# mmbajo/PROBA-V

Measured on AMD Instinct MI355X. Metric: LR-patches/sec fwd+bwd (WDSR-B r12 t9, 16x16, bs128), higher is better.
Workload: dtype f32 (products as 3 scaled-fp16-piece MFMA products, f32 accumulate)

## Files before the change

### proba-v_amd/csrc/kernels_direct.hip

```cpp
#include "probav_common.h"
#include "x6_device.h"

namespace probav {

__device__ __forceinline__ int reflect_idx(int i, int n) {
    i = i < 0 ? -i : i;
    return i >= n ? 2 * n - 2 - i : i;
}

template <int COUT_T, int VEC>
__global__ __launch_bounds__(256) void conv_direct_fwd_kernel(
    ConvGeom g, const float* __restrict__ x, const float* __restrict__ gate, const float* __restrict__ w,
    const float* __restrict__ bias, const float* __restrict__ skip, float* __restrict__ y)
{
    const long nvox = (long)g.N * g.Ho * g.Wo * g.To;
    const long v = (long)blockIdx.x * 256 + threadIdx.x;
    if (v >= nvox) return;
    const int co0 = blockIdx.y * COUT_T;
    long r = v;
    const int t = (int)(r % g.To); r /= g.To;
    const int wo = (int)(r % g.Wo); r /= g.Wo;
    const int h = (int)(r % g.Ho);
    const int n = (int)(r / g.Ho);

// ... 7 lines not shown
        if (g.reflect_hw) ih = reflect_idx(ih, g.Hi);
        else if (ih < 0 || ih >= g.Hi) { pad_h = true; ih = 0; }
        for (int b = 0; b < g.kw; ++b) {
            int iw = wo + b - g.pw;
            bool pad_w = pad_h;
            if (g.reflect_hw) iw = reflect_idx(iw, g.Wi);
            else if (iw < 0 || iw >= g.Wi) { pad_w = true; iw = 0; }
            for (int c = 0; c < g.kt; ++c) {
                int it = t + c - g.pt;
                bool pad = pad_w;
                if (g.reflect_t) it = reflect_idx(it, g.Ti);
                else if (it < 0 || it >= g.Ti) { pad = true; it = 0; }
                const long vin = (((long)n * g.Hi + ih) * g.Wi + iw) * g.Ti + it;
                const float* xp = x + vin * g.Cin;
                const float* gp = gate ? gate + vin * g.Cin : nullptr;
                const float* wp = w + (long)((a * g.kw + b) * g.kt + c) * g.Cin * g.Cout + co0;
                for (int ci = 0; ci < g.Cin; ci += VEC) {
                    float xv[VEC];
                    if constexpr (VEC == 4) {
                        const float4 q = *reinterpret_cast<const float4*>(xp + ci);
                        xv[0] = q.x; xv[1] = q.y; xv[2] = q.z; xv[3] = q.w;
                        if (gp) {
                            const float4 m = *reinterpret_cast<const float4*>(gp + ci);
                            xv[0] = m.x > 0.f ? xv[0] : 0.f; xv[1] = m.y > 0.f ? xv[1] : 0.f;
                            xv[2] = m.z > 0.f ? xv[2] : 0.f; xv[3] = m.w > 0.f ? xv[3] : 0.f;
                        }
                    } else {
                        xv[0] = xp[ci];
                        if (gp) xv[0] = gp[ci] > 0.f ? xv[0] : 0.f;
                    }
#pragma unroll
                    for (int u = 0; u < VEC; ++u) {
                        if (pad) xv[u] = 0.f;
                        const float* wr = wp + (long)(ci + u) * g.Cout;
#pragma unroll
                        for (int j = 0; j < COUT_T; ++j) acc[j] = fmaf(xv[u], wr[j], acc[j]);
                    }
                }
            }
        }
    }
    float* yp = y + v * g.Cout + co0;
    const float* sp = skip ? skip + v * g.Cout + co0 : nullptr;
#pragma unroll
    for (int j = 0; j < COUT_T; ++j) {
        float o = acc[j] + (bias ? bias[co0 + j] : 0.f);
        if (g.relu) o = relu_keep_nan(o);
        if (sp) o += sp[j];
        yp[j] = o;
    }
}

template <int COUT_T>
static int launch_fwd(const ConvGeom& g, const float* x, const float* gate, const float* w, const float* bias,
                      const float* skip, float* y, hipStream_t s)
{
    const long nvox = (long)g.N * g.Ho * g.Wo * g.To;
    dim3 grid((unsigned)((nvox + 255) / 256), (unsigned)(g.Cout / COUT_T));
    const bool vec4 = (g.Cin % 4 == 0) && ((reinterpret_cast<uintptr_t>(x) & 15) == 0) &&
                      (!gate || (reinterpret_cast<uintptr_t>(gate) & 15) == 0);
    if (vec4) hipLaunchKernelGGL((conv_direct_fwd_kernel<COUT_T, 4>), grid, dim3(256), 0, s, g, x, gate, w, bias, skip, y);
    else      hipLaunchKernelGGL((conv_direct_fwd_kernel<COUT_T, 1>), grid, dim3(256), 0, s, g, x, gate, w, bias, skip, y);
    return check_launch("conv_direct_fwd");
}

constexpr int C1_ROWS = 4;
__global__ __launch_bounds__(256) void conv3_cin1_fwd_kernel(ConvGeom g, const float* __restrict__ x, const float* __restrict__ w,
                                                            const float* __restrict__ bias, float* __restrict__ y, unsigned* __restrict__ amax)
{
    extern __shared__ float c1_in[];
    const int tid = threadIdx.x, cg = tid & 7, vs = tid >> 3;
    const int Wp = g.Wi + 2, Tp = g.Ti + 2, nin = 3 * Wp * Tp, nv = g.Wo * g.To;
    float4 wt[27];
#pragma unroll
    for (int k = 0; k < 27; ++k) wt[k] = *reinterpret_cast<const float4*>(w + k * 32 + 4 * cg);
    const float4 b4 = bias ? *reinterpret_cast<const float4*>(bias + 4 * cg) : make_float4(0.f, 0.f, 0.f, 0.f);
    const unsigned mT = 0xffffffffu / (unsigned)g.To + 1u, mTp = 0xffffffffu / (unsigned)Tp + 1u, mWT = 0xffffffffu / (unsigned)(Wp * Tp) + 1u;
    const long nrows = (long)g.N * g.Ho;
    float omax = 0.f;
    int n_prev = -1;
#pragma unroll 1
    for (int r = 0; r < C1_ROWS; ++r) {
        const long R = (long)blockIdx.x * C1_ROWS + r;
        if (R >= nrows) break;
        const int n = (int)(R / g.Ho), h = (int)(R - (long)n * g.Ho);
        if (n != n_prev) { if (amax && n_prev >= 0) amax_commit(omax, amax + n_prev); omax = 0.f; n_prev = n; }
        __syncthreads();
        for (int i = tid; i < nin; i += 256) {
            const int dh = (int)__umulhi((unsigned)i, mWT), rem = i - dh * Wp * Tp;
            const int wp = (int)__umulhi((unsigned)rem, mTp), tp = rem - wp * Tp;
            const int ih = h - 1 + dh, iw = wp - 1, it = tp - 1;
            const bool ok = ih >= 0 && ih < g.Hi && iw >= 0 && iw < g.Wi && it >= 0 && it < g.Ti;
            c1_in[i] = ok ? x[(((long)n * g.Hi + ih) * g.Wi + iw) * g.Ti + it] : 0.f;
        }
        __syncthreads();
        float* yrow = y + ((long)n * g.Ho + h) * nv * 32;
        for (int v = vs; v < nv; v += 32) {
            const int wo = (int)__umulhi((unsigned)v, mT), t = v - wo * g.To;
            const float* ip = c1_in + wo * Tp + t;
            float4 acc = b4;
#pragma unroll
            for (int dh = 0; dh < 3; ++dh)
#pragma unroll
                for (int dw = 0; dw < 3; ++dw)
#pragma unroll
                    for (int dt = 0; dt < 3; ++dt) {
                        const float xv = ip[(dh * Wp + dw) * Tp + dt];
                        const float4 q = wt[(dh * 3 + dw) * 3 + dt];
                        acc.x = fmaf(xv, q.x, acc.x); acc.y = fmaf(xv, q.y, acc.y); acc.z = fmaf(xv, q.z, acc.z); acc.w = fmaf(xv, q.w, acc.w);
                    }
            if (g.relu) { acc.x = relu_keep_nan(acc.x); acc.y = relu_keep_nan(acc.y); acc.z = relu_keep_nan(acc.z); acc.w = relu_keep_nan(acc.w); }
            *reinterpret_cast<float4*>(yrow + (long)v * 32 + 4 * cg) = acc;
            omax = fmaxf(fmaxf(omax, fmaxf(fabsf(acc.x), fabsf(acc.y))), fmaxf(fabsf(acc.z), fabsf(acc.w)));
        }
    }
    if (amax && n_prev >= 0) amax_commit(omax, amax + n_prev);
}

bool conv3d_cin1_forward_supported(const ConvGeom& g)
{
    return g.Cin == 1 && g.Cout == 32 && g.kh == 3 && g.kw == 3 && g.kt == 3 && g.ph == 1 && g.pw == 1 && g.pt == 1 && !g.reflect_hw && !g.reflect_t &&
           g.Ho == g.Hi && g.Wo == g.Wi && g.To == g.Ti && g.To >= 2 && (g.Wi + 2) * (g.Ti + 2) * 3 * sizeof(float) <= 48 * 1024;
}
int conv3d_cin1_forward(const ConvGeom& g, const float* x, const float* w, const float* bias, float* y, unsigned* amax, hipStream_t s)
{
    if (!conv3d_cin1_forward_supported(g)) { set_error("conv3d_cin1_forward: unsupported geometry", hipSuccess); return PROBAV_EINVAL; }
    const long nrows = (long)g.N * g.Ho;
    const size_t lds = (size_t)3 * (g.Wi + 2) * (g.Ti + 2) * sizeof(float);
    hipLaunchKernelGGL(conv3_cin1_fwd_kernel, dim3((unsigned)((nrows + C1_ROWS - 1) / C1_ROWS)), dim3(256), lds, s, g, x, w, bias, y, amax);
    return check_launch("conv3_cin1_fwd");
}

int conv3d_direct_forward(const ConvGeom& g, const float* x, const float* gate, const float* w,
                          const float* bias, const float* skip, float* y, hipStream_t s)
{
    if (g.N <= 0) return PROBAV_OK;
    if (g.Cout % 32 == 0) return launch_fwd<32>(g, x, gate, w, bias, skip, y, s);
    if (g.Cout % 25 == 0) return launch_fwd<25>(g, x, gate, w, bias, skip, y, s);
    if (g.Cout % 9 == 0)  return launch_fwd<9>(g, x, gate, w, bias, skip, y, s);
    if (g.Cout % 4 == 0)  return launch_fwd<4>(g, x, gate, w, bias, skip, y, s);
    return launch_fwd<1>(g, x, gate, w, bias, skip, y, s);
}

bool conv3d_up_forward_supported(const ConvGeom& g)
{
    return g.Cin == 32 && g.Cout == 9 && g.kh == 3 && g.kw == 3 && g.kt == 3 && g.ph == 0 && g.pw == 0 && g.pt == 0 && !g.reflect_hw && !g.reflect_t &&
           g.Ti == 3 && g.To == 1 && g.Ho == g.Hi - 2 && g.Wo == g.Wi - 2 && g.Wo == 16;
}
bool conv3d_up_bwd_data_supported(const ConvGeom& g)
{
    return g.Cin == 9 && g.Cout == 32 && g.kh == 3 && g.kw == 3 && g.kt == 3 && g.ph == 2 && g.pw == 2 && g.pt == 2 && !g.reflect_hw && !g.reflect_t &&
           g.Ti == 1 && g.To == 3 && g.Ho == g.Hi + 2 && g.Wo == g.Wi + 2 && g.Wi <= 30;
}
__global__ __launch_bounds__(256) void conv3_up_fwd_kernel(ConvGeom g, const float* __restrict__ x, const float* __restrict__ w,
                                                          const float* __restrict__ bias, float* __restrict__ y)
{
    extern __shared__ float up_lds[];
    float* sW = up_lds;
    float* sX = sW + 27 * 32 * 9;
    const int tid = threadIdx.x;
    const int rowf = g.Wi * 3 * 32;
    if ((reinterpret_cast<unsigned long>(w) & 15) == 0) {
        for (int i = tid; i < 27 * 32 * 9 / 4; i += 256) reinterpret_cast<float4*>(sW)[i] = reinterpret_cast<const float4*>(w)[i];
    } else {
        for (int i = tid; i < 27 * 32 * 9; i += 256) sW[i] = w[i];
    }
    const int wo = tid >> 4, kp = tid & 15;
    for (int row = blockIdx.x; row < g.N * g.Ho; row += gridDim.x) {
    const int n = row / g.Ho, h = row - n * g.Ho;
    __syncthreads();
    const float4* xr = reinterpret_cast<const float4*>(x + ((long)n * g.Hi + h) * rowf);
    for (int i = tid; i < 3 * rowf / 4; i += 256) reinterpret_cast<float4*>(sX)[i] = xr[i];
    __syncthreads();
    float acc[9];
#pragma unroll
    for (int j = 0; j < 9; ++j) acc[j] = 0.f;
#pragma unroll 2
    for (int q = 0; q < 54; ++q) {
        const int k = kp + 16 * q;
        const int tap = k >> 5, ci = k & 31;
        const int a = tap / 9, bc = tap - 9 * a, b = bc / 3, c = bc - 3 * b;
        const float xv = sX[a * rowf + ((wo + b) * 3 + c) * 32 + ci];
        const float* wr = sW + k * 9;
#pragma unroll
        for (int j = 0; j < 9; ++j) acc[j] = fmaf(xv, wr[j], acc[j]);
    }
#pragma unroll
    for (int j = 0; j < 9; ++j) {
        float v = acc[j];
#pragma unroll
        for (int m = 1; m < 16; m <<= 1) v += __shfl_xor(v, m, 64);
        acc[j] = v;
    }
    if (kp < 9) {
        float o = 0.f;
#pragma unroll
        for (int j = 0; j < 9; ++j) o = kp == j ? acc[j] : o;
        o += bias ? bias[kp] : 0.f;
        if (g.relu) o = relu_keep_nan(o);
        y[(((long)n * g.Ho + h) * g.Wo + wo) * 9 + kp] = o;
    }
    }
}
__global__ __launch_bounds__(256) void conv3_up_bwd_data_kernel(ConvGeom g, const float* __restrict__ dy, const float* __restrict__ wT,
                                                               const float* __restrict__ bias, float* __restrict__ dx, unsigned* __restrict__ amax)
{
    extern __shared__ float up_lds[];
    float* sW = up_lds;
    float* sD = sW + 27 * 9 * 32;
    const int tid = threadIdx.x;
    const int Wp = g.Wi + 4;
    if ((reinterpret_cast<unsigned long>(wT) & 15) == 0) {
        for (int i = tid; i < 27 * 9 * 32 / 4; i += 256) reinterpret_cast<float4*>(sW)[i] = reinterpret_cast<const float4*>(wT)[i];
    } else {
        for (int i = tid; i < 27 * 9 * 32; i += 256) sW[i] = wT[i];
    }
    __shared__ float red[4];
    for (int row = blockIdx.x; row < g.N * g.Ho; row += gridDim.x) {
    const int n = row / g.Ho, h = row - n * g.Ho;
    __syncthreads();
    for (int i = tid; i < 3 * Wp * 9; i += 256) {
        const int a = i / (Wp * 9), r = i - a * Wp * 9, wp = r / 9, co = r - 9 * wp;
        const int ih = h + a - 2, iw = wp - 2;
        sD[i] = (ih >= 0 && ih < g.Hi && iw >= 0 && iw < g.Wi) ? dy[(((long)n * g.Hi + ih) * g.Wi + iw) * 9 + co] : 0.f;
    }
    __syncthreads();
    float omax = 0.f;
    const int items = g.Wo * 3 * 8;
    for (int it = tid; it < items; it += 256) {
        const int cg = it & 7, wt = it >> 3, wo = wt / 3, t = wt - 3 * wo;
        float4 acc = bias ? make_float4(bias[4 * cg], bias[4 * cg + 1], bias[4 * cg + 2], bias[4 * cg + 3]) : make_float4(0.f, 0.f, 0.f, 0.f);
#pragma unroll
        for (int a = 0; a < 3; ++a)
#pragma unroll
            for (int b = 0; b < 3; ++b) {
                const float* dp = sD + (a * Wp + wo + b) * 9;
                const float* wp = sW + (((a * 3 + b) * 3 + (2 - t)) * 9) * 32 + 4 * cg;
#pragma unroll
                for (int co = 0; co < 9; ++co) {
                    const float d = dp[co];
                    const float4 q = *reinterpret_cast<const float4*>(wp + co * 32);
                    acc.x = fmaf(d, q.x, acc.x); acc.y = fmaf(d, q.y, acc.y); acc.z = fmaf(d, q.z, acc.z); acc.w = fmaf(d, q.w, acc.w);
                }
            }
        *reinterpret_cast<float4*>(dx + ((((long)n * g.Ho + h) * g.Wo + wo) * 3 + t) * 32 + 4 * cg) = acc;
        omax = fmaxf(fmaxf(omax, fmaxf(fabsf(acc.x), fabsf(acc.y))), fmaxf(fabsf(acc.z), fabsf(acc.w)));
    }
    if (amax) {
#pragma unroll
        for (int o = 32; o; o >>= 1) omax = fmaxf(omax, __shfl_xor(omax, o, 64));
        if ((tid & 63) == 0) red[tid >> 6] = omax;
        __syncthreads();
        if (tid == 0) {
            const float m = fmaxf(fmaxf(red[0], red[1]), fmaxf(red[2], red[3]));
            atomicMax(amax + n, __float_as_uint(m));
        }
    }
    }
}
int conv3d_up_forward(const ConvGeom& g, const float* x, const float* w, const float* bias, float* y, hipStream_t s)
{
    if (!conv3d_up_forward_supported(g)) { set_error("conv3d_up_forward: unsupported geometry", hipSuccess); return PROBAV_EINVAL; }
    const size_t lds = ((size_t)27 * 32 * 9 + (size_t)3 * g.Wi * 3 * 32) * sizeof(float);
    hipLaunchKernelGGL(conv3_up_fwd_kernel, dim3((unsigned)(g.N * g.Ho < 512 ? g.N * g.Ho : 512)), dim3(256), lds, s, g, x, w, bias, y);
    return check_launch("conv3_up_fwd");
}
int conv3d_up_bwd_data(const ConvGeom& g, const float* dy, const float* wT, const float* bias, float* dx, unsigned* amax, hipStream_t s)
{
    if (!conv3d_up_bwd_data_supported(g)) { set_error("conv3d_up_bwd_data: unsupported geometry", hipSuccess); return PROBAV_EINVAL; }
    const size_t lds = ((size_t)27 * 9 * 32 + (size_t)3 * (g.Wi + 4) * 9) * sizeof(float);
    hipLaunchKernelGGL(conv3_up_bwd_data_kernel, dim3((unsigned)(g.N * g.Ho < 768 ? g.N * g.Ho : 768)), dim3(256), lds, s, g, dy, wT, bias, dx, amax);
    return check_launch("conv3_up_bwd_data");
}

template <int KH, int KW, int KT, int CI_PER>
__global__ __launch_bounds__(256) void conv_direct_wgrad_kernel(
    ConvGeom g, const float* __restrict__ x, const float* __restrict__ dy, const float* __restrict__ gate,
    float* __restrict__ partial, float* __restrict__ partial_b, long vox_per_chunk)
{
    constexpr int TAPS = KH * KW * KT;
    const int tid = threadIdx.x;
    const int co = blockIdx.y * 32 + (tid & 31);
    const bool co_ok = co < g.Cout;
    const int ci0 = (blockIdx.z * 8 + (tid >> 5)) * CI_PER;
    const long nvox = (long)g.N * g.Ho * g.Wo * g.To;
    const long v0 = (long)blockIdx.x * vox_per_chunk;
    const long v1 = v0 + vox_per_chunk < nvox ? v0 + vox_per_chunk : nvox;

    float acc[TAPS][CI_PER];
#pragma unroll
    for (int tp = 0; tp < TAPS; ++tp)
#pragma unroll
        for (int k = 0; k < CI_PER; ++k) acc[tp][k] = 0.f;
    float accb = 0.f;
    const bool vec4 = (CI_PER % 4 == 0) && (g.Cin % 4 == 0) && (ci0 + CI_PER <= g.Cin);

    for (long v = v0; v < v1; ++v) {
        long r = v;
        const int t = (int)(r % g.To); r /= g.To;
        const int wo = (int)(r % g.Wo); r /= g.Wo;
        const int h = (int)(r % g.Ho);
        const int n = (int)(r / g.Ho);
        float d = 0.f;
        if (co_ok) {
            d = dy[v * g.Cout + co];
            if (gate) d = gate[v * g.Cout + co] > 0.f ? d : 0.f;
        }
        accb += d;
#pragma unroll
        for (int a = 0; a < KH; ++a) {
            int ih = h + a - g.ph;
            if (g.reflect_hw) ih = reflect_idx(ih, g.Hi);
            else if (ih < 0 || ih >= g.Hi) continue;
#pragma unroll
            for (int b = 0; b < KW; ++b) {
                int iw = wo + b - g.pw;
                if (g.reflect_hw) iw = reflect_idx(iw, g.Wi);
                else if (iw < 0 || iw >= g.Wi) continue;
#pragma unroll
                for (int c = 0; c < KT; ++c) {
                    int it = t + c - g.pt;
                    if (g.reflect_t) it = reflect_idx(it, g.Ti);
                    else if (it < 0 || it >= g.Ti) continue;
                    const float* xp = x + ((((long)n * g.Hi + ih) * g.Wi + iw) * g.Ti + it) * g.Cin + ci0;
                    const int tp = (a * KW + b) * KT + c;
                    bool done = false;
                    if constexpr (CI_PER % 4 == 0) {
                        if (vec4) {
#pragma unroll
                            for (int k = 0; k < CI_PER; k += 4) {
                                const float4 q = *reinterpret_cast<const float4*>(xp + k);
                                acc[tp][k] = fmaf(q.x, d, acc[tp][k]);
                                acc[tp][k + 1] = fmaf(q.y, d, acc[tp][k + 1]);
                                acc[tp][k + 2] = fmaf(q.z, d, acc[tp][k + 2]);
                                acc[tp][k + 3] = fmaf(q.w, d, acc[tp][k + 3]);
                            }
                            done = true;
                        }
                    }
                    if (!done) {
#pragma unroll
                        for (int k = 0; k < CI_PER; ++k)
                            if (ci0 + k < g.Cin) acc[tp][k] = fmaf(xp[k], d, acc[tp][k]);
                    }
                }
            }
        }
    }
    if (co_ok) {
        float* pp = partial + (long)blockIdx.x * TAPS * g.Cin * g.Cout;
#pragma unroll
        for (int tp = 0; tp < TAPS; ++tp)
#pragma unroll
            for (int k = 0; k < CI_PER; ++k)
                if (ci0 + k < g.Cin) pp[((long)tp * g.Cin + ci0 + k) * g.Cout + co] = acc[tp][k];
        if (blockIdx.z == 0 && (tid >> 5) == 0) partial_b[(long)blockIdx.x * g.Cout + co] = accb;
    }
}

static int sum_partials(const float* p1, float* o1, long n1, const float* p2, float* o2, long n2, int chunks, hipStream_t s)
{
    SlabSumJob jobs[2] = {{p1, o1, n1, (int)n1, chunks}, {p2, o2, n2, (int)n2, chunks}};
    return slab_sum_later(s, jobs, o2 ? 2 : 1);
}


__global__ __launch_bounds__(1024) void wgrad2d_small_kernel(ConvGeom g, const float* __restrict__ x, const float* __restrict__ dy,
                                                            const float* __restrict__ gate, float* __restrict__ partial,
                                                            float* __restrict__ partial_b, int halves)
{
    extern __shared__ float lds2d[];
    const int tid = threadIdx.x, nthr = blockDim.x;
    const int n = blockIdx.x / halves, part = blockIdx.x - n * halves;
    const int r0 = part * g.Ho / halves, r1 = (part + 1) * g.Ho / halves;
    const int nrow_o = r1 - r0, nrow_i = nrow_o + 2;
    float* xs = lds2d;
    float* ds = xs + nrow_i * g.Wi * g.Cin;
    const float* xsrc = x + ((long)n * g.Hi + r0) * g.Wi * g.Cin;
    for (int i = tid; i < nrow_i * g.Wi * g.Cin; i += nthr) xs[i] = xsrc[i];
    const long dbase = ((long)n * g.Ho + r0) * g.Wo * g.Cout;
    for (int i = tid; i < nrow_o * g.Wo * g.Cout; i += nthr) {
        float d = dy[dbase + i];
        if (gate) d = gate[dbase + i] > 0.f ? d : 0.f;
        ds[i] = d;
    }
    __syncthreads();
    const int nout = 9 * g.Cin * g.Cout;
    const long slab = (long)nout + g.Cout;
    float* pp = partial + (long)blockIdx.x * nout;
    if (tid < nout) {
        const int co = tid % g.Cout, rest = tid / g.Cout, ci = rest % g.Cin, tap = rest / g.Cin;
        const int a = tap / 3, b = tap - 3 * a;
        const float* xp = xs + (a * g.Wi + b) * g.Cin + ci;
        const float* dp = ds + co;
        float acc = 0.f;
        for (int h = 0; h < nrow_o; ++h)
            for (int w = 0; w < g.Wo; ++w) acc = fmaf(xp[(h * g.Wi + w) * g.Cin], dp[(h * g.Wo + w) * g.Cout], acc);
        pp[tid] = acc;
    } else if (tid < nout + g.Cout) {
        const int co = tid - nout;
        float acc = 0.f;
        for (int i = 0; i < nrow_o * g.Wo; ++i) acc += ds[i * g.Cout + co];
        partial_b[(long)blockIdx.x * g.Cout + co] = acc;
    }
    (void)slab;
}

static bool small2d(const ConvGeom& g, int& halves, size_t& lds)
{
    if (g.kh != 3 || g.kw != 3 || g.kt != 1 || g.Ti != 1 || g.To != 1 || g.ph || g.pw || g.pt || g.reflect_hw) return false;
    if (9 * g.Cin * g.Cout + g.Cout > 1024 || g.Ho < 2) return false;
    halves = 2;
    const int nrow_o = (g.Ho + 1) / 2 + 1;
    lds = ((size_t)(nrow_o + 2) * g.Wi * g.Cin + (size_t)nrow_o * g.Wo * g.Cout) * sizeof(float);
    return lds <= 64 * 1024;
}

static void wgrad_plan(const ConvGeom& g, int& ci_per, int& gy, int& gz, int& chunks, long& vpc)
{
    const bool k3d = (g.kh == 3 && g.kw == 3 && g.kt == 3);
    const bool k2d = (g.kh == 3 && g.kw == 3 && g.kt == 1);
    if (g.kh == 5) ci_per = 1;
    else if (k3d) ci_per = g.Cin >= 4 ? 4 : 1;
// ... 312 lines not shown
```

### proba-v_amd/csrc/kernels_loss.hip

```cpp
#include "probav_common.h"
#include "reduce_device.h"

namespace probav {

__device__ __forceinline__ double corrected(double p, double bias, double m) { return (p + bias) * m; }
__device__ __forceinline__ double residual(double h, double p, double bias, double m) { return h - corrected(p, bias, m); }

struct Crop {
    const float* H; const uint8_t* M; const float* P;
    int S, border, L, i, j;
    __device__ __forceinline__ bool clear(int r, int c) const { return M[(i + r) * S + j + c] != 0; }
    __device__ __forceinline__ float hr(int r, int c) const { return H[(i + r) * S + j + c]; }
    __device__ __forceinline__ float pred(int r, int c) const { return P[(border + r) * S + border + c]; }
    __device__ __forceinline__ double m(int r, int c) const { return clear(r, c) ? 1.0 : 0.0; }
    __device__ __forceinline__ double residual(int r, int c, double bias) const { return probav::residual((double)hr(r, c), (double)pred(r, c), bias, m(r, c)); }
};
__device__ __forceinline__ Crop crop_at(const float* hr, const uint8_t* mask, const float* pred, int b, int S, int border, int i, int j)
{
    const long o = (long)b * S * S;
    return Crop{hr + o, mask + o, pred + o, S, border, S - 2 * border, i, j};
}
__device__ __forceinline__ Crop crop_of_shift(const float* hr, const uint8_t* mask, const float* pred, int b, int S, int border, int sft)
{
    const int ns = 2 * border + 1, i = sft / ns;
    return crop_at(hr, mask, pred, b, S, border, i, sft - i * ns);
}

__device__ __forceinline__ void crop_walk(const Crop& x, int tid, double& cnt, double& dsum)
{
    cnt = 0.0; dsum = 0.0;
    for (int k = tid; k < x.L * x.L; k += 256) {
        const int r = k / x.L, c = k - r * x.L;
        const float m = x.clear(r, c) ? 1.f : 0.f;
        cnt += (double)m;
        dsum += (double)(x.hr(r, c) - x.pred(r, c) * m);
    }
}
__device__ __forceinline__ double crop_bias(const Crop& x, int tid, double* red, double& cnt)
{
    double dsum;
    crop_walk(x, tid, cnt, dsum);
    cnt = block_sum(cnt, red, tid);
    dsum = block_sum(dsum, red, tid);
    return dsum / cnt;
}

struct FirstMin {
    double best = 1e300;
    int arg = 0;
    __device__ __forceinline__ void take(double v, int sft) { if (v < best) { best = v; arg = sft; } }
    __device__ __forceinline__ double value() const { return best < 1e300 ? best : __builtin_nan(""); }
};

__global__ __launch_bounds__(256) void shift_loss_fwd_kernel(
    const float* __restrict__ hr, const uint8_t* __restrict__ mask, const float* __restrict__ pred, int S, int border,
    double* __restrict__ cand)
{
    const int b = blockIdx.x, i = blockIdx.y, lane = threadIdx.x & 63, wave = threadIdx.x >> 6;
    const int L = S - 2 * border, ns = 2 * border + 1, nshift = ns * ns;
    for (int j = wave; j < ns; j += 4) {
        const int sft = i * ns + j;
        const Crop x = crop_at(hr, mask, pred, b, S, border, i, j);
        constexpr int U = 4;
        const int n = L * L;
        double cnt = 0.0, dsum = 0.0;
        for (int k0 = lane; k0 < n; k0 += 64 * U) {
            float m[U], h[U], q[U];
#pragma unroll
            for (int u = 0; u < U; ++u) {
                const int k = k0 + 64 * u < n ? k0 + 64 * u : k0;
                const int r = k / L, c = k - r * L;
                m[u] = x.clear(r, c) ? 1.f : 0.f;
                h[u] = x.hr(r, c);
                q[u] = x.pred(r, c);
            }
#pragma unroll
            for (int u = 0; u < U; ++u)
                if (k0 + 64 * u < n) { cnt += (double)m[u]; dsum += (double)(h[u] - q[u] * m[u]); }
        }
        cnt = wave_sum(cnt); dsum = wave_sum(dsum);
        const double bias = dsum / cnt;
        double s1 = 0.0, s2 = 0.0;
        for (int k0 = lane; k0 < n; k0 += 64 * U) {
            float h[U], q[U]; bool mk[U];
#pragma unroll
            for (int u = 0; u < U; ++u) {
                const int k = k0 + 64 * u < n ? k0 + 64 * u : k0;
                const int r = k / L, c = k - r * L;
                mk[u] = x.clear(r, c);
                h[u] = x.hr(r, c);
                q[u] = x.pred(r, c);
            }
#pragma unroll
            for (int u = 0; u < U; ++u)
                if (k0 + 64 * u < n) {
                    const double e = residual((double)h[u], (double)q[u], bias, mk[u] ? 1.0 : 0.0);
                    s1 += fabs(e);
                    s2 += e * e;
                }
        }
        s1 = wave_sum(s1) / cnt; s2 = wave_sum(s2) / cnt;
        if (lane == 0) { cand[((long)b * nshift + sft) * 2] = s1; cand[((long)b * nshift + sft) * 2 + 1] = s2; }
    }
}

__global__ __launch_bounds__(64) void batch_mean_kernel(const float* __restrict__ a, const float* __restrict__ b2,
                                                       float* __restrict__ ma, float* __restrict__ mb, int n)
{
    double s1 = 0.0, s2 = 0.0;
    for (int i = threadIdx.x; i < n; i += 64) { s1 += (double)a[i]; s2 += (double)b2[i]; }
    s1 = wave_sum(s1); s2 = wave_sum(s2);
    if (threadIdx.x == 0) { *ma = (float)(s1 / n); *mb = (float)(s2 / n); }
}

__device__ __forceinline__ void shift_select_sample(const double* __restrict__ cand, int b, int nshift, float max_val, float* __restrict__ l1_out,
                                                    float* __restrict__ l2_out, float* __restrict__ cpsnr_out, int* __restrict__ arg_l1,
                                                    int* __restrict__ arg_l2, float& l1, float& l2)
{
    const double2* c = reinterpret_cast<const double2*>(cand) + (long)b * nshift;
    FirstMin m1, m2;
#pragma unroll 7
    for (int sft = 0; sft < nshift; ++sft) {
        const double2 v = c[sft];
        m1.take(v.x, sft);
        m2.take(v.y, sft);
    }
    l1_out[b] = l1 = (float)m1.value();
    l2_out[b] = l2 = (float)m2.value();
    cpsnr_out[b] = (float)(10.0 * log10((double)max_val * (double)max_val / m2.value()));
    arg_l1[b] = m1.arg;
    arg_l2[b] = m2.arg;
}
__global__ __launch_bounds__(1024) void shift_select_mean_kernel(const double* __restrict__ cand, int B, int nshift, float max_val,
                                                                float* __restrict__ l1_out, float* __restrict__ l2_out, float* __restrict__ cpsnr_out,
                                                                int* __restrict__ arg_l1, int* __restrict__ arg_l2, float* __restrict__ ma, float* __restrict__ mb)
{
    __shared__ float sl1[1024], sl2[1024];
    const int b = threadIdx.x;
    if (b < B) shift_select_sample(cand, b, nshift, max_val, l1_out, l2_out, cpsnr_out, arg_l1, arg_l2, sl1[b], sl2[b]);
    __syncthreads();
    if (threadIdx.x < 64) {
        double s1 = 0.0, s2 = 0.0;
        for (int i = threadIdx.x; i < B; i += 64) { s1 += (double)sl1[i]; s2 += (double)sl2[i]; }
        s1 = wave_sum(s1); s2 = wave_sum(s2);
        if (threadIdx.x == 0) { *ma = (float)(s1 / B); *mb = (float)(s2 / B); }
    }
}

__global__ __launch_bounds__(64) void shift_select_kernel(const double* __restrict__ cand, int B, int nshift, float max_val,
                                                         float* __restrict__ l1_out, float* __restrict__ l2_out, float* __restrict__ cpsnr_out,
                                                         int* __restrict__ arg_l1, int* __restrict__ arg_l2)
{
    const int b = blockIdx.x * 64 + threadIdx.x;
    float l1, l2;
    if (b < B) shift_select_sample(cand, b, nshift, max_val, l1_out, l2_out, cpsnr_out, arg_l1, arg_l2, l1, l2);
}

int shift_loss_forward(const float* hr, const uint8_t* mask, const float* pred, int B, int S, int border,
                       float* l1, float* l2, float* cpsnr, int* arg_l1, int* arg_l2, float* mean_l1, float* mean_l2,
                       float max_val, hipStream_t s)
{
    if (B <= 0 || border < 0 || S <= 2 * border) { set_error("shift_loss_forward: bad shape (size must exceed 2 * border)", hipSuccess); return PROBAV_EINVAL; }
    const int ns = 2 * border + 1;
    static double* cand = nullptr;
    static size_t cand_n = 0;
    const size_t need = (size_t)B * ns * ns * 2;
    if (need > cand_n) {
        if (cand) (void)hipFree(cand);
        cand = nullptr; cand_n = 0;
        hipError_t err = hipMalloc((void**)&cand, need * sizeof(double));
        if (err != hipSuccess) { set_error("shift_loss_forward: scratch allocation", err); return PROBAV_EHIP; }
        cand_n = need;
    }
    hipLaunchKernelGGL(shift_loss_fwd_kernel, dim3(B, ns), dim3(256), 0, s, hr, mask, pred, S, border, cand);
    if (B <= 1024) {
        hipLaunchKernelGGL(shift_select_mean_kernel, dim3(1), dim3((unsigned)((B + 63) / 64 * 64)), 0, s, cand, B, ns * ns, max_val, l1, l2, cpsnr, arg_l1, arg_l2, mean_l1, mean_l2);
        return check_launch("shift_loss_forward");
    }
    hipLaunchKernelGGL(shift_select_kernel, dim3((unsigned)((B + 63) / 64)), dim3(64), 0, s, cand, B, ns * ns, max_val, l1, l2, cpsnr, arg_l1, arg_l2);
    hipLaunchKernelGGL(batch_mean_kernel, dim3(1), dim3(64), 0, s, l1, l2, mean_l1, mean_l2, B);
    return check_launch("shift_loss_forward");
}

__global__ __launch_bounds__(256) void shift_loss_bwd_kernel(
    const float* __restrict__ hr, const uint8_t* __restrict__ mask, const float* __restrict__ pred,
    const int* __restrict__ arg, int S, int border, int which, const float* __restrict__ upstream, float inv_b,
    float* __restrict__ dpred)
{
    const float scale = (upstream ? upstream[0] : 1.f) * inv_b;
    const int b = blockIdx.x, tid = threadIdx.x, lane = tid & 63, wave = tid >> 6;
    const Crop x = crop_of_shift(hr, mask, pred, b, S, border, arg[b]);
    const int L = x.L;
    float* G = dpred + (long)b * S * S;
    __shared__ double red[2][4];
    double cnt, dsum;
    crop_walk(x, tid, cnt, dsum);
    cnt = wave_sum(cnt); dsum = wave_sum(dsum);
    if (lane == 0) { red[0][wave] = cnt; red[1][wave] = dsum; }
    __syncthreads();
    cnt = red[0][0] + red[0][1] + red[0][2] + red[0][3];
    dsum = red[1][0] + red[1][1] + red[1][2] + red[1][3];
    const double bias = dsum / cnt;
    __syncthreads();
    double ssum = 0.0;
    for (int k = tid; k < L * L; k += 256) {
        const int r = k / L, c = k - r * L;
        const double e = x.residual(r, c, bias);
        const double sg = which == 1 ? sign_keep_nan(e) : 2.0 * e;
        ssum += sg * x.m(r, c);
    }
    ssum = wave_sum(ssum);
    if (lane == 0) red[0][wave] = ssum;
    __syncthreads();
    ssum = red[0][0] + red[0][1] + red[0][2] + red[0][3];
    for (int k = tid; k < S * S; k += 256) {
        const int Y = k / S, X = k - Y * S, r = Y - border, c = X - border;
        float gk = 0.f;
        if (r >= 0 && r < L && c >= 0 && c < L) {
            const double e = x.residual(r, c, bias);
            const double sg = which == 1 ? sign_keep_nan(e) : 2.0 * e;
            gk = (float)(-(x.m(r, c) / cnt) * (sg - ssum / cnt) * (double)scale);
        }
        G[k] = gk;
    }
}
int shift_loss_backward(const float* hr, const uint8_t* mask, const float* pred, const int* arg, int B, int S,
                        int border, int which, const float* upstream, float* dpred, hipStream_t s)
{
    if (which != 1 && which != 2) { set_error("shift_loss_backward: which must be 1 (L1) or 2 (L2)", hipSuccess); return PROBAV_EINVAL; }
    if (B <= 0 || border < 0 || S <= 2 * border) { set_error("shift_loss_backward: bad shape (size must exceed 2 * border)", hipSuccess); return PROBAV_EINVAL; }
    hipLaunchKernelGGL(shift_loss_bwd_kernel, dim3(B), dim3(256), 0, s, hr, mask, pred, arg, S, border, which, upstream, 1.0f / (float)B, dpred);
    return check_launch("shift_loss_backward");
}

__device__ __forceinline__ int mirror(int i, int n) { return i < 0 ? -i : (i >= n ? 2 * n - 2 - i : i); }

__device__ __forceinline__ void sobel_at(const float* sD, int k, int L, double& gy, double& gx)
{
    const int r = k / L, c = k - r * L;
    const int r0 = mirror(r - 1, L) * L, r1 = r * L, r2 = mirror(r + 1, L) * L;
    const int c0 = mirror(c - 1, L), c2 = mirror(c + 1, L);
    gy = ((double)sD[r2 + c0] + 2.0 * sD[r2 + c] + sD[r2 + c2]) - ((double)sD[r0 + c0] + 2.0 * sD[r0 + c] + sD[r0 + c2]);
    gx = ((double)sD[r0 + c2] + 2.0 * sD[r1 + c2] + sD[r2 + c2]) - ((double)sD[r0 + c0] + 2.0 * sD[r1 + c0] + sD[r2 + c0]);
}

__global__ __launch_bounds__(256) void shift_l1edge_fwd_kernel(
    const float* __restrict__ hr, const uint8_t* __restrict__ mask, const float* __restrict__ pred, int S, int border, float pi,
    float* __restrict__ loss_out, int* __restrict__ arg_out)
{
    extern __shared__ float sD[];
    __shared__ double red[4];
    const int b = blockIdx.x, tid = threadIdx.x;
    const int L = S - 2 * border, ns = 2 * border + 1, nshift = ns * ns;
    FirstMin best;
    for (int sft = 0; sft < nshift; ++sft) {
        const Crop x = crop_of_shift(hr, mask, pred, b, S, border, sft);
        double cnt;
        const double bias = crop_bias(x, tid, red, cnt);
        double s1 = 0.0;
        for (int k = tid; k < L * L; k += 256) {
            const int r = k / L, c = k - r * L;
            const double e = x.residual(r, c, bias);
            sD[k] = (float)e;
            s1 += fabs(e);
        }
        s1 = block_sum(s1, red, tid);
        double sg = 0.0;
        for (int k = tid; k < L * L; k += 256) {
            double gy, gx;
            sobel_at(sD, k, L, gy, gx);
            sg += fabs(gy) + fabs(gx);
        }
        sg = block_sum(sg, red, tid);
        best.take(((double)pi * s1 + (1.0 - (double)pi) * sg) / cnt, sft);
    }
    if (tid == 0) { loss_out[b] = (float)best.value(); arg_out[b] = best.arg; }
}

__global__ __launch_bounds__(256) void shift_l1edge_bwd_kernel(
    const float* __restrict__ hr, const uint8_t* __restrict__ mask, const float* __restrict__ pred, const int* __restrict__ arg,
    int S, int border, float pi, const float* __restrict__ upstream, float inv_b, float* __restrict__ dpred)
{
    extern __shared__ float sm[];
    __shared__ double red[4];
    const int b = blockIdx.x, tid = threadIdx.x;
    const int L = S - 2 * border, Lp = L + 2;
    float* sD = sm;
    float* sY = sD + L * L;
    float* sX = sY + L * L;
    float* sG = sX + L * L;
    const float scale = (upstream ? upstream[0] : 1.f) * inv_b;
    const Crop x = crop_of_shift(hr, mask, pred, b, S, border, arg[b]);
    float* G = dpred + (long)b * S * S;
    double cnt;
    const double bias = crop_bias(x, tid, red, cnt);
    for (int k = tid; k < L * L; k += 256) {
        const int r = k / L, c = k - r * L;
        sD[k] = (float)x.residual(r, c, bias);
    }
    __syncthreads();
    for (int k = tid; k < L * L; k += 256) {
        double gy, gx;
        sobel_at(sD, k, L, gy, gx);
        sY[k] = (float)sign_keep_nan(gy);
        sX[k] = (float)sign_keep_nan(gx);
    }
    __syncthreads();
    for (int k = tid; k < Lp * Lp; k += 256) {
        const int u = k / Lp - 1, v = k - (k / Lp) * Lp - 1;
        float acc = 0.f;
#pragma unroll
        for (int a = 0; a < 3; ++a)
#pragma unroll
            for (int bb = 0; bb < 3; ++bb) {
                const int qr = u - (a - 1), qc = v - (bb - 1);
                if (qr < 0 || qr >= L || qc < 0 || qc >= L) continue;
                const float ky = (a == 0 ? -1.f : (a == 2 ? 1.f : 0.f)) * (bb == 1 ? 2.f : 1.f);
                const float kx = (bb == 0 ? -1.f : (bb == 2 ? 1.f : 0.f)) * (a == 1 ? 2.f : 1.f);
                acc += ky * sY[qr * L + qc] + kx * sX[qr * L + qc];
            }
        sG[k] = acc;
    }
    __syncthreads();
    double gm = 0.0;
    for (int k = tid; k < L * L; k += 256) {
        const int r = k / L, c = k - r * L;
        float acc = 0.f;
// ... 260 lines not shown
```

Baseline: 21450.

## Register-block up-conv kernels and stage shift-loss tiles in LDS

The up-conv forward kernel now gives each block 4 output rows, one per wave. It stages the needed input rows with padded LDS strides, and each lane computes 4 output columns so every weight load is reused. The up-conv backward-data kernel computes two adjacent output columns per item to reuse weight loads. The shift-loss forward kernel copies the HR/pred/mask strip into LDS, uses up to 16 waves per block, and replaces per-pixel divisions with incremental row/column indexing. The costs are more registers, larger LDS and blocks, and a one-shot grid in place of the persistent loop.

```diff
diff --git a/proba-v_amd/csrc/kernels_direct.hip b/proba-v_amd/csrc/kernels_direct.hip
--- a/proba-v_amd/csrc/kernels_direct.hip
+++ b/proba-v_amd/csrc/kernels_direct.hip
@@ -183,54 +183,78 @@
     return g.Cin == 9 && g.Cout == 32 && g.kh == 3 && g.kw == 3 && g.kt == 3 && g.ph == 2 && g.pw == 2 && g.pt == 2 && !g.reflect_hw && !g.reflect_t &&
            g.Ti == 1 && g.To == 3 && g.Ho == g.Hi + 2 && g.Wo == g.Wi + 2 && g.Wi <= 30;
 }
-__global__ __launch_bounds__(256) void conv3_up_fwd_kernel(ConvGeom g, const float* __restrict__ x, const float* __restrict__ w,
-                                                          const float* __restrict__ bias, float* __restrict__ y)
+constexpr int UP_ROWS = 4;
+constexpr int UP_XS = 3 * 32 + 16;
+__global__ __launch_bounds__(64 * UP_ROWS) void conv3_up_fwd_kernel(ConvGeom g, const float* __restrict__ x, const float* __restrict__ w,
+                                                                   const float* __restrict__ bias, float* __restrict__ y)
 {
     extern __shared__ float up_lds[];
     float* sW = up_lds;
     float* sX = sW + 27 * 32 * 9;
-    const int tid = threadIdx.x;
-    const int rowf = g.Wi * 3 * 32;
+    const int tid = threadIdx.x, wave = tid >> 6, lane = tid & 63;
+    const int ngrp = (g.Ho + UP_ROWS - 1) / UP_ROWS;
+    const int n = blockIdx.x / ngrp, h0 = (blockIdx.x - n * ngrp) * UP_ROWS;
+    const int rows_in = (g.Ho - h0 < UP_ROWS ? g.Ho - h0 : UP_ROWS) + 2;
     if ((reinterpret_cast<unsigned long>(w) & 15) == 0) {
-        for (int i = tid; i < 27 * 32 * 9 / 4; i += 256) reinterpret_cast<float4*>(sW)[i] = reinterpret_cast<const float4*>(w)[i];
+        for (int i = tid; i < 27 * 32 * 9 / 4; i += 64 * UP_ROWS) reinterpret_cast<float4*>(sW)[i] = reinterpret_cast<const float4*>(w)[i];
     } else {
-        for (int i = tid; i < 27 * 32 * 9; i += 256) sW[i] = w[i];
-    }
-    const int wo = tid >> 4, kp = tid & 15;
-    for (int row = blockIdx.x; row < g.N * g.Ho; row += gridDim.x) {
-    const int n = row / g.Ho, h = row - n * g.Ho;
-    __syncthreads();
-    const float4* xr = reinterpret_cast<const float4*>(x + ((long)n * g.Hi + h) * rowf);
-    for (int i = tid; i < 3 * rowf / 4; i += 256) reinterpret_cast<float4*>(sX)[i] = xr[i];
-    __syncthreads();
-    float acc[9];
-#pragma unroll
-    for (int j = 0; j < 9; ++j) acc[j] = 0.f;
+        for (int i = tid; i < 27 * 32 * 9; i += 64 * UP_ROWS) sW[i] = w[i];
+    }
+    {
+        const float4* xr = reinterpret_cast<const float4*>(x + ((long)n * g.Hi + h0) * g.Wi * 96);
+        const int n4 = rows_in * g.Wi * 24;
+        for (int i = tid; i < n4; i += 64 * UP_ROWS) {
+            const int col = i / 24, part = i - col * 24;
+            reinterpret_cast<float4*>(sX)[col * (UP_XS / 4) + part] = xr[i];
+        }
+    }
+    __syncthreads();
+    const int h = h0 + wave;
+    if (h >= g.Ho) return;
+    const int kp = lane & 15, wq = lane >> 4;
+    float acc[4][9];
+#pragma unroll
+    for (int m = 0; m < 4; ++m)
+#pragma unroll
+        for (int j = 0; j < 9; ++j) acc[m][j] = 0.f;
+    const float* xw = sX + (wave * g.Wi + wq) * UP_XS;
 #pragma unroll 2
     for (int q = 0; q < 54; ++q) {
         const int k = kp + 16 * q;
         const int tap = k >> 5, ci = k & 31;
         const int a = tap / 9, bc = tap - 9 * a, b = bc / 3, c = bc - 3 * b;
-        const float xv = sX[a * rowf + ((wo + b) * 3 + c) * 32 + ci];
+        const float* xp = xw + (a * g.Wi + b) * UP_XS + c * 32 + ci;
         const float* wr = sW + k * 9;
-#pragma unroll
-        for (int j = 0; j < 9; ++j) acc[j] = fmaf(xv, wr[j], acc[j]);
-    }
-#pragma unroll
-    for (int j = 0; j < 9; ++j) {
-        float v = acc[j];
-#pragma unroll
-        for (int m = 1; m < 16; m <<= 1) v += __shfl_xor(v, m, 64);
-        acc[j] = v;
-    }
+        float wv[9];
+#pragma unroll
+        for (int j = 0; j < 9; ++j) wv[j] = wr[j];
+#pragma unroll
+        for (int m = 0; m < 4; ++m) {
+            const float xv = xp[4 * m * UP_XS];
+#pragma unroll
+            for (int j = 0; j < 9; ++j) acc[m][j] = fmaf(xv, wv[j], acc[m][j]);
+        }
+    }
+#pragma unroll
+    for (int m = 0; m < 4; ++m)
+#pragma unroll
+        for (int j = 0; j < 9; ++j) {
+            float v = acc[m][j];
+#pragma unroll
+            for (int o = 1; o < 16; o <<= 1) v += __shfl_xor(v, o, 64);
+            acc[m][j] = v;
+        }
     if (kp < 9) {
-        float o = 0.f;
-#pragma unroll
-        for (int j = 0; j < 9; ++j) o = kp == j ? acc[j] : o;
-        o += bias ? bias[kp] : 0.f;
-        if (g.relu) o = relu_keep_nan(o);
-        y[(((long)n * g.Ho + h) * g.Wo + wo) * 9 + kp] = o;
-    }
+        const float bv = bias ? bias[kp] : 0.f;
+#pragma unroll
+        for (int m = 0; m < 4; ++m) {
+            float o = 0.f;
+#pragma unroll
+            for (int j = 0; j < 9; ++j) o = kp == j ? acc[m][j] : o;
+            o += bv;
+            if (g.relu) o = relu_keep_nan(o);
+            y[(((long)n * g.Ho + h) * g.Wo + wq + 4 * m) * 9 + kp] = o;
+        }
     }
 }
 __global__ __launch_bounds__(256) void conv3_up_bwd_data_kernel(ConvGeom g, const float* __restrict__ dy, const float* __restrict__ wT,
@@ -257,11 +281,13 @@
     }
     __syncthreads();
     float omax = 0.f;
-    const int items = g.Wo * 3 * 8;
+    const int wpairs = (g.Wo + 1) >> 1, items = wpairs * 3 * 8;
     for (int it = tid; it < items; it += 256) {
-        const int cg = it & 7, wt = it >> 3, wo = wt / 3, t = wt - 3 * wo;
-        float4 acc = bias ? make_float4(bias[4 * cg], bias[4 * cg + 1], bias[4 * cg + 2], bias[4 * cg + 3]) : make_float4(0.f, 0.f, 0.f, 0.f);
-#pragma unroll
+        const int cg = it & 7, wt = it >> 3, wq = wt / 3, t = wt - 3 * wq, wo = 2 * wq;
+        const bool two = wo + 1 < g.Wo;
+        const float4 b4 = bias ? make_float4(bias[4 * cg], bias[4 * cg + 1], bias[4 * cg + 2], bias[4 * cg + 3]) : make_float4(0.f, 0.f, 0.f, 0.f);
+        float4 acc = b4, acc1 = b4;
+#pragma unroll 1
         for (int a = 0; a < 3; ++a)
 #pragma unroll
             for (int b = 0; b < 3; ++b) {
@@ -269,13 +295,19 @@
                 const float* wp = sW + (((a * 3 + b) * 3 + (2 - t)) * 9) * 32 + 4 * cg;
 #pragma unroll
                 for (int co = 0; co < 9; ++co) {
-                    const float d = dp[co];
+                    const float d = dp[co], d1 = dp[9 + co];
                     const float4 q = *reinterpret_cast<const float4*>(wp + co * 32);
                     acc.x = fmaf(d, q.x, acc.x); acc.y = fmaf(d, q.y, acc.y); acc.z = fmaf(d, q.z, acc.z); acc.w = fmaf(d, q.w, acc.w);
+                    acc1.x = fmaf(d1, q.x, acc1.x); acc1.y = fmaf(d1, q.y, acc1.y); acc1.z = fmaf(d1, q.z, acc1.z); acc1.w = fmaf(d1, q.w, acc1.w);
                 }
             }
-        *reinterpret_cast<float4*>(dx + ((((long)n * g.Ho + h) * g.Wo + wo) * 3 + t) * 32 + 4 * cg) = acc;
+        float* op = dx + ((((long)n * g.Ho + h) * g.Wo + wo) * 3 + t) * 32 + 4 * cg;
+        *reinterpret_cast<float4*>(op) = acc;
         omax = fmaxf(fmaxf(omax, fmaxf(fabsf(acc.x), fabsf(acc.y))), fmaxf(fabsf(acc.z), fabsf(acc.w)));
+        if (two) {
+            *reinterpret_cast<float4*>(op + 3 * 32) = acc1;
+            omax = fmaxf(fmaxf(omax, fmaxf(fabsf(acc1.x), fabsf(acc1.y))), fmaxf(fabsf(acc1.z), fabsf(acc1.w)));
+        }
     }
     if (amax) {
 #pragma unroll
@@ -292,14 +324,15 @@
 int conv3d_up_forward(const ConvGeom& g, const float* x, const float* w, const float* bias, float* y, hipStream_t s)
 {
     if (!conv3d_up_forward_supported(g)) { set_error("conv3d_up_forward: unsupported geometry", hipSuccess); return PROBAV_EINVAL; }
-    const size_t lds = ((size_t)27 * 32 * 9 + (size_t)3 * g.Wi * 3 * 32) * sizeof(float);
-    hipLaunchKernelGGL(conv3_up_fwd_kernel, dim3((unsigned)(g.N * g.Ho < 512 ? g.N * g.Ho : 512)), dim3(256), lds, s, g, x, w, bias, y);
-    return check_launch("conv3_up_fwd");
+    const size_t lds = ((size_t)27 * 32 * 9 + (size_t)(UP_ROWS + 2) * g.Wi * UP_XS) * sizeof(float);
+    const long grid = (long)g.N * ((g.Ho + UP_ROWS - 1) / UP_ROWS);
+    if (grid > 0x7fffffffL) { set_error("conv3d_up_forward: batch too large", hipSuccess); return PROBAV_EINVAL; }
+    return launch_lds<conv3_up_fwd_kernel>("conv3_up_fwd", dim3((unsigned)grid), dim3(64 * UP_ROWS), lds, s, g, x, w, bias, y);
 }
 int conv3d_up_bwd_data(const ConvGeom& g, const float* dy, const float* wT, const float* bias, float* dx, unsigned* amax, hipStream_t s)
 {
     if (!conv3d_up_bwd_data_supported(g)) { set_error("conv3d_up_bwd_data: unsupported geometry", hipSuccess); return PROBAV_EINVAL; }
-    const size_t lds = ((size_t)27 * 9 * 32 + (size_t)3 * (g.Wi + 4) * 9) * sizeof(float);
+    const size_t lds = ((size_t)27 * 9 * 32 + ((size_t)3 * (g.Wi + 4) + 1) * 9) * sizeof(float);
     hipLaunchKernelGGL(conv3_up_bwd_data_kernel, dim3((unsigned)(g.N * g.Ho < 768 ? g.N * g.Ho : 768)), dim3(256), lds, s, g, dy, wT, bias, dx, amax);
     return check_launch("conv3_up_bwd_data");
 }
diff --git a/proba-v_amd/csrc/kernels_loss.hip b/proba-v_amd/csrc/kernels_loss.hip
--- a/proba-v_amd/csrc/kernels_loss.hip
+++ b/proba-v_amd/csrc/kernels_loss.hip
@@ -52,27 +52,61 @@
     __device__ __forceinline__ double value() const { return best < 1e300 ? best : __builtin_nan(""); }
 };
 
-__global__ __launch_bounds__(256) void shift_loss_fwd_kernel(
+constexpr int SHIFT_FWD_MAX_WAVES = 16;
+static size_t shift_fwd_tile_bytes(int S, int border) { return (size_t)(S - 2 * border) * S * (2 * sizeof(float) + 1); }
+template <bool TILE>
+__global__ __launch_bounds__(64 * SHIFT_FWD_MAX_WAVES) void shift_loss_fwd_kernel(
     const float* __restrict__ hr, const uint8_t* __restrict__ mask, const float* __restrict__ pred, int S, int border,
     double* __restrict__ cand)
 {
-    const int b = blockIdx.x, i = blockIdx.y, lane = threadIdx.x & 63, wave = threadIdx.x >> 6;
-    const int L = S - 2 * border, ns = 2 * border + 1, nshift = ns * ns;
-    for (int j = wave; j < ns; j += 4) {
+    extern __shared__ float shift_tile[];
+    const int b = blockIdx.x, i = blockIdx.y, lane = threadIdx.x & 63, wave = threadIdx.x >> 6, nwave = blockDim.x >> 6;
+    const int L = S - 2 * border, ns = 2 * border + 1, nshift = ns * ns, n = L * L, LS = L * S;
+    constexpr int U = 4;
+    const float* tH = shift_tile;
+    const float* tP = shift_tile + LS;
+    const uint8_t* tM = reinterpret_cast<const uint8_t*>(shift_tile + 2 * LS);
+    if constexpr (TILE) {
+        const long o = (long)b * S * S;
+        const float* gH = hr + o + (long)i * S;
+        const float* gP = pred + o + (long)border * S;
+        const uint8_t* gM = mask + o + (long)i * S;
+        float* wH = shift_tile;
+        float* wP = shift_tile + LS;
+        uint8_t* wM = reinterpret_cast<uint8_t*>(shift_tile + 2 * LS);
+        const int nthr = blockDim.x;
+        for (int k0 = threadIdx.x; k0 < LS; k0 += U * nthr) {
+            float h[U], q[U]; uint8_t m[U];
+#pragma unroll
+            for (int u = 0; u < U; ++u) {
+                const int k = k0 + u * nthr < LS ? k0 + u * nthr : k0;
+                h[u] = gH[k]; q[u] = gP[k]; m[u] = gM[k];
+            }
+#pragma unroll
+            for (int u = 0; u < U; ++u)
+                if (k0 + u * nthr < LS) { const int k = k0 + u * nthr; wH[k] = h[u]; wP[k] = q[u]; wM[k] = m[u]; }
+        }
+        __syncthreads();
+    }
+    const int dq = 64 / L, dc = 64 - dq * L, r_lane = lane / L, c_lane = lane - r_lane * L;
+    for (int j = wave; j < ns; j += nwave) {
         const int sft = i * ns + j;
         const Crop x = crop_at(hr, mask, pred, b, S, border, i, j);
-        constexpr int U = 4;
-        const int n = L * L;
+        auto pixel = [&](int r, int c, float& m, float& h, float& q) {
+            if constexpr (TILE) { const int a = r * S + c; m = tM[a + j] != 0 ? 1.f : 0.f; h = tH[a + j]; q = tP[a + border]; }
+            else { m = x.clear(r, c) ? 1.f : 0.f; h = x.hr(r, c); q = x.pred(r, c); }
+        };
         double cnt = 0.0, dsum = 0.0;
+        int r = r_lane, c = c_lane;
         for (int k0 = lane; k0 < n; k0 += 64 * U) {
             float m[U], h[U], q[U];
+            const int r0 = r, c0 = c;
 #pragma unroll
             for (int u = 0; u < U; ++u) {
-                const int k = k0 + 64 * u < n ? k0 + 64 * u : k0;
-                const int r = k / L, c = k - r * L;
-                m[u] = x.clear(r, c) ? 1.f : 0.f;
-                h[u] = x.hr(r, c);
-                q[u] = x.pred(r, c);
+                const bool in = k0 + 64 * u < n;
+                pixel(in ? r : r0, in ? c : c0, m[u], h[u], q[u]);
+                c += dc; r += dq;
+                if (c >= L) { c -= L; ++r; }
             }
 #pragma unroll
             for (int u = 0; u < U; ++u)
@@ -81,20 +115,21 @@
         cnt = wave_sum(cnt); dsum = wave_sum(dsum);
         const double bias = dsum / cnt;
         double s1 = 0.0, s2 = 0.0;
+        r = r_lane; c = c_lane;
         for (int k0 = lane; k0 < n; k0 += 64 * U) {
-            float h[U], q[U]; bool mk[U];
+            float m[U], h[U], q[U];
+            const int r0 = r, c0 = c;
 #pragma unroll
             for (int u = 0; u < U; ++u) {
-                const int k = k0 + 64 * u < n ? k0 + 64 * u : k0;
-                const int r = k / L, c = k - r * L;
-                mk[u] = x.clear(r, c);
-                h[u] = x.hr(r, c);
-                q[u] = x.pred(r, c);
+                const bool in = k0 + 64 * u < n;
+                pixel(in ? r : r0, in ? c : c0, m[u], h[u], q[u]);
+                c += dc; r += dq;
+                if (c >= L) { c -= L; ++r; }
             }
 #pragma unroll
             for (int u = 0; u < U; ++u)
                 if (k0 + 64 * u < n) {
-                    const double e = residual((double)h[u], (double)q[u], bias, mk[u] ? 1.0 : 0.0);
+                    const double e = residual((double)h[u], (double)q[u], bias, (double)m[u]);
                     s1 += fabs(e);
                     s2 += e * e;
                 }
@@ -172,7 +207,12 @@
         if (err != hipSuccess) { set_error("shift_loss_forward: scratch allocation", err); return PROBAV_EHIP; }
         cand_n = need;
     }
-    hipLaunchKernelGGL(shift_loss_fwd_kernel, dim3(B, ns), dim3(256), 0, s, hr, mask, pred, S, border, cand);
+    {
+        const dim3 block(64u * (unsigned)(ns < SHIFT_FWD_MAX_WAVES ? ns : SHIFT_FWD_MAX_WAVES));
+        const size_t tile = shift_fwd_tile_bytes(S, border);
+        if (tile <= LDS_DEFAULT) hipLaunchKernelGGL(shift_loss_fwd_kernel<true>, dim3(B, ns), block, tile, s, hr, mask, pred, S, border, cand);
+        else hipLaunchKernelGGL(shift_loss_fwd_kernel<false>, dim3(B, ns), block, 0, s, hr, mask, pred, S, border, cand);
+    }
     if (B <= 1024) {
         hipLaunchKernelGGL(shift_select_mean_kernel, dim3(1), dim3((unsigned)((B + 63) / 64 * 64)), 0, s, cand, B, ns * ns, max_val, l1, l2, cpsnr, arg_l1, arg_l2, mean_l1, mean_l2);
         return check_launch("shift_loss_forward");
```

Measured after the change: 21590, median of 6. No clear change (+0.7%).
